# agnusmaximus/DistributedMNIST

Measured on AMD Instinct MI355X. Metric: images/sec (whole node), MNIST CNN sync-SGD, higher is better.
Workload: dtype bf16; 1 GPU; model=lenet, global_batch=1024, parallelism=dp1, mode=full_sync, mode_requested=full_sync, grad_dtype=fp32

## Files before the change

csrc/bindings.cpp:

```cpp

#include <torch/extension.h>
#include <ATen/hip/HIPContext.h>
#include <hip/hip_runtime.h>

#include "kernels.h"

namespace {

#define CHECK_BF16(t) TORCH_CHECK((t).scalar_type() == at::kBFloat16, #t " must be bf16")
#define CHECK_F32(t) TORCH_CHECK((t).scalar_type() == at::kFloat, #t " must be fp32")
#define CHECK_CONTIG(t) TORCH_CHECK((t).is_contiguous(), #t " must be contiguous")
#define CHECK_CUDA(t) TORCH_CHECK((t).is_cuda(), #t " must be on GPU")

const unsigned short* bf16_ptr(const torch::Tensor& t) {
  return reinterpret_cast<const unsigned short*>(t.data_ptr());
}
unsigned short* bf16_mut(torch::Tensor& t) {
  return reinterpret_cast<unsigned short*>(t.data_ptr());
}

hipStream_t cur_stream() {
  return at::hip::getCurrentHIPStream().stream();
}

int cdiv(int a, int b) { return (a + b - 1) / b; }

int pick_splitk(int mtiles, int ntiles, int ksteps) {
  int tiles = mtiles * ntiles;
  if (tiles >= 256 || ksteps <= 1) return 1;
  int want = std::min(ksteps, std::max(1, 512 / tiles));
  return want;
}

int dw_tr_level() {
  static int v = [] {
    const char* e = getenv("DMNIST_DW_TR");
    return e ? atoi(e) : 1;
  }();
  return v;
}
bool dw_tr_enabled() { return dw_tr_level() != 0; }

bool conv2_dw_slab_route(int H, int W, int Cin, int Cout) {
  return conv2_dw_slab_supported(H, W, Cin, Cout) && dw_tr_enabled() &&
         conv2_dw_slab_enabled() && !getenv("DMNIST_DW_SPREAD");
}

torch::Tensor linear_act_fwd_impl(torch::Tensor x, torch::Tensor w,
                                  torch::Tensor b, bool relu, double p_keep,
                                  int64_t seed, int64_t offset,
                                  const long* offset_dev,
                                  const c10::optional<torch::Tensor>& wT) {
  CHECK_CUDA(x); CHECK_BF16(x); CHECK_CONTIG(x);
  CHECK_BF16(w); CHECK_CONTIG(w);
  CHECK_F32(b); CHECK_CONTIG(b);
  int M = x.size(0), K = x.size(1), N = w.size(1);
  TORCH_CHECK(w.size(0) == K, "w/x shape mismatch");
  auto y = torch::empty({M, N}, x.options());
  GemmParams p{};
  p.A = bf16_ptr(x);
  p.bias = b.data_ptr<float>();
  p.C = y.data_ptr(); p.amax = nullptr;
  p.M = M; p.N = N; p.K = K;
  p.lda = K; p.ldc = N;
  p.splitk = 1;
  p.p_keep = (float)p_keep; p.seed = (uint64_t)seed; p.offset = (uint64_t)offset;
  p.offset_dev = offset_dev;
  bool drop = p_keep < 1.0;
  TORCH_CHECK(!drop || relu, "dropout path requires relu epilogue");
  int g128 = cdiv(M, 128) * cdiv(N, 128);
  bool big = g128 >= 512;
  if (const char* e = getenv("DMNIST_FC_TILE")) big = atoi(e) >= 128;
  auto s = cur_stream();
  bool bt = wT.has_value() && wT->defined();
  int tiles64 = cdiv(M, 64) * cdiv(N, 64);
  int ksteps = cdiv(K, 64);
  if (!big && tiles64 < 256 && ksteps >= 16 &&
      !getenv("DMNIST_FC_NOSPLIT")) {
    int sk = std::min(ksteps, std::max(2, 512 / tiles64));
    auto acc = torch::empty({(int64_t)sk, (int64_t)M, (int64_t)N},
                            x.options().dtype(at::kFloat));
    p.C = acc.data_ptr();
    p.splitk = sk;
    if (bt) {
      CHECK_BF16((*wT)); CHECK_CONTIG((*wT));
      TORCH_CHECK(wT->size(0) == N && wT->size(1) == K, "wT shape mismatch");
      p.B = bf16_ptr(*wT); p.ldb = K;
      gemm_fwd_slices_64_bt(p, s);
    } else {
      p.B = bf16_ptr(w); p.ldb = N;
      gemm_fwd_slices_64(p, s);
    }
    launch_fwd_epilogue(acc.data_ptr<float>(), b.data_ptr<float>(),
                        bf16_mut(y), M, N, sk, relu ? 1 : 0, (float)p_keep,
                        (uint64_t)seed, (uint64_t)offset, offset_dev, s);
    return y;
  }
  if (bt) {
    CHECK_BF16((*wT)); CHECK_CONTIG((*wT));
    TORCH_CHECK(wT->size(0) == N && wT->size(1) == K, "wT shape mismatch");
    p.B = bf16_ptr(*wT); p.ldb = K;
    if (drop) (big ? gemm_fwd_drop_128_bt : gemm_fwd_drop_64_bt)(p, s);
    else if (relu) (big ? gemm_fwd_relu_128_bt : gemm_fwd_relu_64_bt)(p, s);
    else (big ? gemm_fwd_bias_128_bt : gemm_fwd_bias_64_bt)(p, s);
  } else {
    p.B = bf16_ptr(w); p.ldb = N;
    if (drop) (big ? gemm_fwd_drop_128 : gemm_fwd_drop_64)(p, s);
    else if (relu) (big ? gemm_fwd_relu_128 : gemm_fwd_relu_64)(p, s);
    else (big ? gemm_fwd_bias_128 : gemm_fwd_bias_64)(p, s);
  }
  return y;
}

torch::Tensor linear_act_fwd(torch::Tensor x, torch::Tensor w, torch::Tensor b,
                             bool relu, double p_keep, int64_t seed,
                             int64_t offset,
                             c10::optional<torch::Tensor> wT) {
  return linear_act_fwd_impl(x, w, b, relu, p_keep, seed, offset, nullptr, wT);
// ... 24 lines not shown
  CHECK_F32(db); CHECK_CONTIG(db);
  torch::Tensor dyeff;
  bool mask = relu || p_keep < 1.0;
  if (mask) {
    dyeff = torch::empty_like(dy);
    launch_relu_drop_bwd(bf16_ptr(dy), bf16_ptr(y), bf16_mut(dyeff),
                         db.data_ptr<float>(), B, N,
                         (float)(1.0 / p_keep), 1, s);
  } else {
    dyeff = dy;
    launch_relu_drop_bwd(bf16_ptr(dy), bf16_ptr(y), bf16_mut(dyeff),
                         db.data_ptr<float>(), B, N, 1.0f, 0, s);
  }
  if (!dw.defined())
    dw = torch::zeros({K, N}, x.options().dtype(at::kFloat));
  CHECK_F32(dw); CHECK_CONTIG(dw);
  {
    GemmParams p{};
    p.A = bf16_ptr(x); p.B = bf16_ptr(dyeff);
    p.C = dw.data_ptr();
    p.M = K; p.N = N; p.K = B;
    p.lda = K;
    p.ldb = N; p.ldc = N;
    if (dw_tr_enabled() && K % 8 == 0 && N % 64 == 0) {
      int bn = (N % 128 == 0) ? 128 : 64;
      p.splitk = pick_splitk(cdiv(K, 128), cdiv(N, bn), cdiv(B, 32));
      (bn == 128 ? gemm_dw_tr_128 : gemm_dw_tr_64)(p, s);
    } else {
      bool big = cdiv(K, 128) * cdiv(N, 128) >= 128;
      int bm = big ? 128 : 64;
      p.splitk = pick_splitk(cdiv(K, bm), cdiv(N, bm), cdiv(B, 32));
      (big ? gemm_dw_128 : gemm_dw_64)(p, s);
    }
  }
  torch::Tensor dx;
  if (need_dx) {
    dx = torch::empty({B, K}, x.options());
    GemmParams p{};
    p.A = bf16_ptr(dyeff); p.B = bf16_ptr(w);
    p.C = dx.data_ptr();
    p.M = B; p.N = K; p.K = N;
    p.lda = N; p.ldb = N; p.ldc = K;
    p.splitk = 1;
    bool big = cdiv(B, 128) * cdiv(K, 128) >= 128;
    (big ? gemm_dx_128 : gemm_dx_64)(p, s);
  } else {
    dx = torch::empty({0}, x.options());
  }
  return {dx, dw, db};
}

std::vector<torch::Tensor> linear_act_bwd(torch::Tensor dy, torch::Tensor x,
                                          torch::Tensor w, torch::Tensor y,
                                          bool relu, double p_keep,
                                          bool need_dx) {
  return linear_act_bwd_impl(dy, x, w, y, relu, p_keep, need_dx,
// ... 156 lines not shown
                      double p_keep, torch::Tensor db_out) {
  CHECK_CUDA(dy); CHECK_BF16(dy); CHECK_CONTIG(dy);
  CHECK_F32(db_out); CHECK_CONTIG(db_out);
  int B = dy.size(0), N = dy.size(1);
  auto s = cur_stream();
  bool mask = relu || p_keep < 1.0;
  torch::Tensor dyeff = mask ? torch::empty_like(dy) : dy;
  launch_relu_drop_bwd(bf16_ptr(dy), mask ? bf16_ptr(y) : bf16_ptr(dy),
                       bf16_mut(dyeff), db_out.data_ptr<float>(), B, N,
                       (float)(1.0 / p_keep), mask ? 1 : 0, s);
  return dyeff;
}

void linear_dw_into(torch::Tensor x, torch::Tensor dyeff,
                    torch::Tensor dw_out) {
  CHECK_BF16(x); CHECK_CONTIG(x); CHECK_BF16(dyeff); CHECK_CONTIG(dyeff);
  CHECK_F32(dw_out);
  int B = x.size(0), K = x.size(1), N = dyeff.size(1);
  GemmParams p{};
  p.A = bf16_ptr(x); p.B = bf16_ptr(dyeff);
  p.C = dw_out.data_ptr();
  p.M = K; p.N = N; p.K = B;
  p.lda = K; p.ldb = N; p.ldc = N;
  if (dw_tr_enabled() && K % 8 == 0 && N % 64 == 0) {
    int bn = (N % 128 == 0) ? 128 : 64;
    p.splitk = pick_splitk(cdiv(K, 128), cdiv(N, bn), cdiv(B, 32));
    (bn == 128 ? gemm_dw_tr_128 : gemm_dw_tr_64)(p, cur_stream());
    return;
  }
  bool big = cdiv(K, 128) * cdiv(N, 128) >= 128;
  int bm = big ? 128 : 64;
  p.splitk = pick_splitk(cdiv(K, bm), cdiv(N, bm), cdiv(B, 32));
  (big ? gemm_dw_128 : gemm_dw_64)(p, cur_stream());
}

torch::Tensor linear_dx(torch::Tensor dyeff, torch::Tensor w) {
  CHECK_BF16(dyeff); CHECK_CONTIG(dyeff); CHECK_BF16(w); CHECK_CONTIG(w);
  int B = dyeff.size(0), N = dyeff.size(1), K = w.size(0);
  auto dx = torch::empty({B, K}, dyeff.options());
  GemmParams p{};
  p.A = bf16_ptr(dyeff); p.B = bf16_ptr(w);
  p.C = dx.data_ptr();
  p.M = B; p.N = K; p.K = N;
  p.lda = N; p.ldb = N; p.ldc = K;
  p.splitk = 1;
  bool big = cdiv(B, 128) * cdiv(K, 128) >= 128;
  (big ? gemm_dx_128 : gemm_dx_64)(p, cur_stream());
  return dx;
}

torch::Tensor linear_dx_unpool(torch::Tensor dyeff, torch::Tensor w,
                               torch::Tensor amax, torch::Tensor db_out,
                               int64_t Ho, int64_t Wo, int64_t C) {
  CHECK_BF16(dyeff); CHECK_CONTIG(dyeff); CHECK_BF16(w); CHECK_CONTIG(w);
  int B = dyeff.size(0), N = dyeff.size(1), K = w.size(0);
  TORCH_CHECK(K == Ho * Wo * C, "linear_dx_unpool: K != Ho*Wo*C");
  auto dact = torch::empty({B, 2 * (int)Ho, 2 * (int)Wo, (int)C},
                           dyeff.options());
  GemmParams p{};
  p.A = bf16_ptr(dyeff); p.B = bf16_ptr(w);
  p.C = dact.data_ptr();
  p.M = B; p.N = K; p.K = N;
  p.lda = N; p.ldb = N; p.ldc = K;
  p.splitk = 1;
  p.CHo = Ho; p.CWo = Wo; p.Cout = C;
  p.amax = amax.data_ptr<uint8_t>();
  p.db = db_out.defined() ? db_out.data_ptr<float>() : nullptr;
  bool big = cdiv(B, 128) * cdiv(K, 128) >= 512;
  (big ? gemm_dx_unpool_128 : gemm_dx_unpool_64)(p, cur_stream());
  return dact;
}

torch::Tensor linear_dx_mask(torch::Tensor dyeff, torch::Tensor w,
                             torch::Tensor actm, torch::Tensor db_out,
                             double p_keep) {
  CHECK_BF16(dyeff); CHECK_CONTIG(dyeff); CHECK_BF16(w); CHECK_CONTIG(w);
  CHECK_BF16(actm); CHECK_CONTIG(actm);
  int B = dyeff.size(0), N = dyeff.size(1), K = w.size(0);
  TORCH_CHECK(actm.size(0) == B && actm.size(1) == K, "actm shape mismatch");
  auto dx = torch::empty({B, K}, dyeff.options());
  GemmParams p{};
  p.A = bf16_ptr(dyeff); p.B = bf16_ptr(w);
  p.C = dx.data_ptr();
  p.M = B; p.N = K; p.K = N;
  p.lda = N; p.ldb = N; p.ldc = K;
  p.splitk = 1;
  p.p_keep = (float)(1.0 / p_keep);
  p.actm = bf16_ptr(actm);
  p.db = db_out.defined() ? db_out.data_ptr<float>() : nullptr;
  bool big = cdiv(B, 128) * cdiv(K, 128) >= 128;
  (big ? gemm_dx_mask_128 : gemm_dx_mask_64)(p, cur_stream());
// ... 389 lines not shown
}

PYBIND11_MODULE(TORCH_EXTENSION_NAME, m) {
  m.def("linear_act_fwd", &linear_act_fwd, "fused linear+bias+relu+dropout",
        py::arg("x"), py::arg("w"), py::arg("b"), py::arg("relu"),
        py::arg("p_keep"), py::arg("seed"), py::arg("offset"),
        py::arg("wT") = c10::nullopt);
  m.def("transpose_bf16", &transpose_bf16, "bf16 2-D transpose (wT refresh)");
  m.def("transpose_bf16_batch_adv", &transpose_bf16_batch_adv,
        "batched transposes + fused device step/LR advance (graph tail)");
  m.def("transpose_bf16_batch", &transpose_bf16_batch,
        "up to 4 transposes in one launch");
  m.def("mask_db", &mask_db, "relu/dropout grad mask + bias-grad column sums");
  m.def("linear_dw_into", &linear_dw_into, "dW = x^T dyeff into bucket view");
  m.def("linear_dx", &linear_dx, "dx = dyeff @ W^T");
  m.def("linear_dx_mask", &linear_dx_mask,
        "dx GEMM with fused relu/dropout mask + bias-grad column sums",
        py::arg("dyeff"), py::arg("w"), py::arg("actm"), py::arg("db_out"),
        py::arg("p_keep"));
  m.def("linear_dx_unpool", &linear_dx_unpool,
        "dx GEMM fused with maxpool2x2 backward scatter + conv db",
        py::arg("dyeff"), py::arg("w"), py::arg("amax"),
        py::arg("db_out"), py::arg("Ho"), py::arg("Wo"), py::arg("C"));
  m.def("pool_scatter", &pool_scatter, "maxpool bwd scatter + conv db");
  m.def("conv_dw_into", &conv_dw_into, "conv dW into bucket view");
  m.def("conv1_dw_pooled", &conv1_dw_pooled,
        "conv1 dW+db from the pooled gradient (pool bwd fused, no dact1)",
        py::arg("x"), py::arg("dyp"), py::arg("am"),
        py::arg("dw_out"), py::arg("db_out"));
  m.def("conv1_dw_group", [](int64_t NB) {
          return (int64_t)conv1_mfma_dw_group((int)NB);
        }, "images per block the MFMA conv1 dW launcher picks for batch NB");
  m.def("conv2_dw_group", [](int64_t NB) {
          return (int64_t)conv2_dw_group((int)NB);
        }, "images per block the slab conv2 dW launcher picks for batch NB");
  m.def("conv_dx", &conv_dx, "conv dX");
  m.def("linear_act_bwd", &linear_act_bwd, "linear backward (dx, dw, db)");
  m.def("linear_act_bwd_into", &linear_act_bwd_into,
        "linear backward accumulating dw/db into bucket views");
  m.def("conv_pool_fwd", &conv_pool_fwd, "fused conv5x5+bias+relu+maxpool",
        py::arg("x"), py::arg("w"), py::arg("b"), py::arg("wT") = c10::nullopt);
  m.def("conv_pool_bwd", &conv_pool_bwd, "conv+pool backward (dx, dw, db)");
  m.def("conv_pool_bwd_into", &conv_pool_bwd_into,
        "conv backward accumulating dw/db into bucket views");
  m.def("softmax_xent_fwd", &softmax_xent_fwd, "fused softmax-CE (+grad, +optional fc2 db, +optional acc-mean scale)",
        py::arg("logits"), py::arg("labels"),
// ... 51 lines not shown
```

csrc/dw_tr.hip:

```cpp

#include "common.h"
#include "kernels.h"

#define NT 256

__device__ __align__(16) unsigned short g_zero_page[8];

enum { AM_PLAIN = 0, AM_CONV5 = 1 };

template <int BN, int AMODE, int TBM = 128, int TBK = 64, int NBUF = 2>
__global__ __launch_bounds__(NT) void dw_tr_kernel(GemmParams p) {
  static_assert(TBK % 32 == 0, "TBK in 32-k MFMA halves");
  static_assert(NBUF == 2 || NBUF == 3, "2-buf overlap or 3-buf glds span");
  constexpr int WM = TBM / 2, WN = BN / 2;
  constexpr int MI = WM / 16, NI = WN / 16;
  constexpr int AQ = TBM * TBK / 2048;
  constexpr int BQ = BN * TBK / 2048;
  constexpr int ALPR = TBM / 8;
  constexpr int BLPR = BN / 8;
  __shared__ __align__(16) ushort_t Aimg[NBUF][TBK][TBM];
  __shared__ __align__(16) ushort_t Bimg[NBUF][TBK][BN];

  const int tid = threadIdx.x;
  const int lane = tid & 63;
  const int wave = tid >> 6;
  const int wr = wave >> 1, wc = wave & 1;

  int gx = (p.M + TBM - 1) / TBM;
  int gy = (p.N + BN - 1) / BN;
  int total = gx * gy * p.splitk;
  int flat = blockIdx.x;
  int q8 = total / 8, r8 = total % 8;
  int xcd = flat % 8, pos = flat / 8;
  int flat2 = (xcd < r8 ? xcd * (q8 + 1) : r8 * (q8 + 1) + (xcd - r8) * q8) + pos;
  const int m0 = (flat2 % gx) * TBM;
  int rest = flat2 / gx;
  const int n0 = (rest % gy) * BN;
  const int bz = rest / gy;

  int ksteps_total = (p.K + TBK - 1) / TBK;
  int steps_per = (ksteps_total + p.splitk - 1) / p.splitk;
  int kbeg = bz * steps_per * TBK;
  int kend = min(p.K, kbeg + steps_per * TBK);
  int nt = (kend - kbeg + TBK - 1) / TBK;
  if (nt < 0) nt = 0;

  f32x4 acc[MI][NI];
#pragma unroll
  for (int mi = 0; mi < MI; ++mi)
#pragma unroll
    for (int ni = 0; ni < NI; ++ni) acc[mi][ni] = f32x4{0.f, 0.f, 0.f, 0.f};

  int amc[AQ];
  bool am_ok[AQ];
  int akh[AQ], akw[AQ], aci[AQ];
#pragma unroll
  for (int q = 0; q < AQ; ++q) {
    int rt = (wave * AQ + q) * (512 / TBM) + lane / ALPR;
    int xs = (rt ^ (rt >> 4)) & (ALPR - 1);
    amc[q] = m0 + ((lane % ALPR) ^ xs) * 8;
    am_ok[q] = amc[q] < p.M;
    if (AMODE == AM_CONV5) {
      int khkw = amc[q] / p.Cin;
      aci[q] = amc[q] % p.Cin;
      akh[q] = khkw / 5 - 2;
      akw[q] = khkw % 5 - 2;
    } else {
      akh[q] = akw[q] = aci[q] = 0;
    }
  }
  int bnc[BQ];
  bool bn_ok[BQ];
#pragma unroll
  for (int q = 0; q < BQ; ++q) {
    int rt = (wave * BQ + q) * (512 / BN) + lane / BLPR;
    int xs = (rt ^ (rt >> 3)) & (BLPR - 1);
    bnc[q] = n0 + ((lane % BLPR) ^ xs) * 8;
    bn_ok[q] = bnc[q] < p.N;
  }

  int aw[AQ], ah[AQ], an[AQ];
  int dw64 = 0, dh64 = 0, dn64 = 0;
// ... 41 lines not shown
    for (int q = 0; q < BQ; ++q) {
      int gi = wave * BQ + q;
      int row0 = gi * (512 / BN);
      int k = kt + row0 + lane / BLPR;
      const ushort_t* src = (k < kend && bn_ok[q])
                                ? p.B + (size_t)k * p.ldb + bnc[q]
                                : g_zero_page;
      glds16(src, &Bimg[buf][row0][0]);
    }
  };

  const int slot_r = (lane & 15) >> 2;
  const int slot_c = (lane & 3) * 4;
  const int kgrp = (lane >> 4) * 8;

  const auto compute = [&](int buf) {
    unsigned abase = (unsigned)(uintptr_t)&Aimg[buf][0][0];
    unsigned bbase = (unsigned)(uintptr_t)&Bimg[buf][0][0];
#pragma unroll
    for (int kh2 = 0; kh2 < TBK / 32; ++kh2) {
      int krow = kh2 * 32 + kgrp + slot_r;
      short8 af[MI], bf[NI];
      const auto aswz = [&](int r, int cb) {
        int xs = (r ^ (r >> 4)) & (ALPR - 1);
        return abase + (unsigned)(r * (TBM * 2) + (((cb >> 4) ^ xs) << 4) +
                                  (cb & 15));
      };
      const auto bswz = [&](int r, int cb) {
        int xs = (r ^ (r >> 3)) & (BLPR - 1);
        return bbase + (unsigned)(r * (BN * 2) + (((cb >> 4) ^ xs) << 4) +
                                  (cb & 15));
      };
      uint2 ar[MI][2], br[NI][2];
#pragma unroll
      for (int mi = 0; mi < MI; ++mi) {
        int cb = (wr * WM + mi * 16 + slot_c) * 2;
        ar[mi][0] = tr16_issue(aswz(krow, cb));
        ar[mi][1] = tr16_issue(aswz(krow + 4, cb));
      }
#pragma unroll
      for (int ni = 0; ni < NI; ++ni) {
        int cb = (wc * WN + ni * 16 + slot_c) * 2;
        br[ni][0] = tr16_issue(bswz(krow, cb));
        br[ni][1] = tr16_issue(bswz(krow + 4, cb));
      }
#pragma unroll
      for (int mi = 0; mi < MI; ++mi) af[mi] = pack_wait(ar[mi][0], ar[mi][1]);
#pragma unroll
      for (int ni = 0; ni < NI; ++ni) bf[ni] = pack_wait(br[ni][0], br[ni][1]);
#pragma unroll
      for (int mi = 0; mi < MI; ++mi)
#pragma unroll
        for (int ni = 0; ni < NI; ++ni)
          acc[mi][ni] = __builtin_amdgcn_mfma_f32_16x16x32_bf16(
              af[mi], bf[ni], acc[mi][ni], 0, 0, 0);
    }
  };

  constexpr int INFLIGHT = AQ + BQ;
  if (NBUF == 3) {
    if (nt > 0) issue(0, kbeg);
    if (nt > 1) {
      issue(1 % NBUF, kbeg + TBK);
      asm volatile("s_waitcnt vmcnt(%0)" ::"i"(INFLIGHT) : "memory");
    } else {
      asm volatile("s_waitcnt vmcnt(0)" ::: "memory");
    }
    __builtin_amdgcn_s_barrier();
    for (int t = 0; t < nt; ++t) {
      if (t + 2 < nt) issue((t + 2) % NBUF, kbeg + (t + 2) * TBK);
      compute(t % NBUF);
      if (t + 2 < nt)
        asm volatile("s_waitcnt vmcnt(%0)" ::"i"(INFLIGHT) : "memory");
      else
        asm volatile("s_waitcnt vmcnt(0)" ::: "memory");
      __builtin_amdgcn_s_barrier();
    }
  } else {
    int cur = 0;
    if (nt > 0) issue(0, kbeg);
    asm volatile("s_waitcnt vmcnt(0)" ::: "memory");
    __syncthreads();
    for (int t = 0; t < nt; ++t) {
      if (t + 1 < nt) issue(cur ^ 1, kbeg + (t + 1) * TBK);
      compute(cur);
      __syncthreads();
      cur ^= 1;
    }
  }

  const int frow = (lane >> 4) * 4;
  const int fcol = lane & 15;
  float* outp = reinterpret_cast<float*>(p.C);
  if (p.offset) outp += (size_t)(bz & 15) * p.M * p.ldc;
#pragma unroll
  for (int mi = 0; mi < MI; ++mi) {
#pragma unroll
    for (int ni = 0; ni < NI; ++ni) {
      int gc = n0 + wc * WN + ni * 16 + fcol;
      if (gc >= p.N) continue;
#pragma unroll
      for (int r = 0; r < 4; ++r) {
        int gr = m0 + wr * WM + mi * 16 + frow + r;
        if (gr >= p.M) continue;
        atomicAdd(outp + (size_t)gr * p.ldc + gc, acc[mi][ni][r]);
      }
    }
  }
}

static inline int cdiv_h(int a, int b) { return (a + b - 1) / b; }

void conv_dw_tr(const GemmParams& p, hipStream_t s) {
  static int tbm = [] {
    const char* e = getenv("DMNIST_DW_TBM");
    return e ? atoi(e) : 128;
  }();
  static int tbk = [] {
    const char* e = getenv("DMNIST_DW_TBK");
    return e ? atoi(e) : 32;
  }();
  dim3 grid(cdiv_h(p.M, tbm >= 256 ? 256 : 128) * cdiv_h(p.N, 64) * p.splitk);
  if (tbm >= 256)
    hipLaunchKernelGGL((dw_tr_kernel<64, AM_CONV5, 256>), grid, dim3(NT), 0,
                       s, p);
  else if (tbk <= 32 && getenv("DMNIST_DW_SPAN"))
    hipLaunchKernelGGL((dw_tr_kernel<64, AM_CONV5, 128, 32, 3>), grid,
                       dim3(NT), 0, s, p);
  else if (tbk <= 32)
    hipLaunchKernelGGL((dw_tr_kernel<64, AM_CONV5, 128, 32>), grid, dim3(NT),
                       0, s, p);
  else
    hipLaunchKernelGGL((dw_tr_kernel<64, AM_CONV5, 128>), grid, dim3(NT), 0,
                       s, p);
}

void gemm_dw_tr_128(const GemmParams& p, hipStream_t s) {
  dim3 grid(cdiv_h(p.M, 128) * cdiv_h(p.N, 128) * p.splitk);
  hipLaunchKernelGGL((dw_tr_kernel<128, AM_PLAIN>), grid, dim3(NT), 0, s, p);
}

void gemm_dw_tr_64(const GemmParams& p, hipStream_t s) {
  dim3 grid(cdiv_h(p.M, 128) * cdiv_h(p.N, 64) * p.splitk);
  hipLaunchKernelGGL((dw_tr_kernel<64, AM_PLAIN>), grid, dim3(NT), 0, s, p);
}
```

csrc/gemm_tile.hip:

```cpp

#include "common.h"
#include "kernels.h"

enum AMode {
  A_N = 0,
  A_T = 1,
  A_CONV_FWD = 2,
  A_CONV1_FWD = 3,
  A_CONV_DX = 4,
  A_CONV_DW = 5,
};
enum BMode {
  B_KMAJ = 0,
  B_NMAJ = 1,
  B_CONV_DX_W = 2,
};
enum Epi { EPI_NONE = 0, EPI_BIAS = 1, EPI_BIAS_RELU = 2, EPI_BIAS_RELU_DROP = 3,
           EPI_POOL = 4, EPI_UNPOOL = 5, EPI_MASK_DB = 6 };
enum OutKind { OUT_BF16 = 0, OUT_F32_ATOMIC = 1, OUT_F32_SLICES = 2 };

#define NTHREADS 256
#define BK 64
#define LDK (BK + 8)

DEV short8 loadRow8(const ushort_t* p, int vcnt) {
  short8 v;
  if (vcnt >= 8 && ((uintptr_t)p & 15) == 0) {
    v = *reinterpret_cast<const short8*>(p);
  } else {
#pragma unroll
    for (int j = 0; j < 8; ++j) v[j] = (j < vcnt) ? (short)p[j] : (short)0;
  }
  return v;
}

DEV bool decode_pool_m(const GemmParams& p, int m, int& n, int& oy, int& ox) {
  int q = m >> 2, pos = m & 3;
  int wo = q % p.CWo;
  int t = q / p.CWo;
  int ho = t % p.CHo;
  n = t / p.CHo;
  oy = ho * 2 + (pos >> 1);
// ... 153 lines not shown
    if (BMODE == B_KMAJ) {
      int kk = c / (BN / 8);
      int j0 = (c % (BN / 8)) * 8;
#pragma unroll
      for (int e = 0; e < 8; ++e) Bs[j0 + e][kk] = regs[j][e];
    } else {
      int i = c / (BK / 8);
      int kc = (c % (BK / 8)) * 8;
      *reinterpret_cast<short8*>(&Bs[i][kc]) = regs[j];
    }
  }
}

template <int BM, int BN, int AMODE, int BMODE, int EPI, int OUT, int PIPE,
          int SWZ = 0>
__global__ __launch_bounds__(NTHREADS)
void gemm_tile_kernel(GemmParams p) {
  constexpr int WM = BM / 2, WN = BN / 2;
  constexpr int MI = WM / 16, NI = WN / 16;
  constexpr int CHA = (BM * BK / 8) / NTHREADS;
  constexpr int CHB = (BN * BK / 8) / NTHREADS;
  constexpr int DB = (PIPE == 1) ? 2 : 1;
  static_assert(CHA >= 1 && CHB >= 1, "tile too small for 256 threads");
  __shared__ __align__(16) ushort_t As[DB][BM][LDK];
  __shared__ __align__(16) ushort_t Bs[DB][BN][LDK];
  constexpr bool HAS_DB = (EPI == EPI_UNPOOL || EPI == EPI_MASK_DB);
  __shared__ float dbred[HAS_DB ? BN : 1];
  if (HAS_DB && threadIdx.x < BN) dbred[threadIdx.x] = 0.f;

  const int tid = threadIdx.x;
  const int lane = tid & 63;
  const int wave = tid >> 6;
  const int wr = wave >> 1, wc = wave & 1;
  int bx = blockIdx.x, by = blockIdx.y, bz = blockIdx.z;
  if (SWZ) {
    int gx = (p.M + BM - 1) / BM;
    int gy = (p.N + BN - 1) / BN;
    int total = gx * gy * p.splitk;
    int flat = blockIdx.x;
    int q = total / 8, r = total % 8;
    int xcd = flat % 8, pos = flat / 8;
    int flat2 = (xcd < r ? xcd * (q + 1) : r * (q + 1) + (xcd - r) * q) + pos;
    bx = flat2 % gx;
    int rest = flat2 / gx;
    by = rest % gy;
    bz = rest / gy;
  }
  const int m0 = bx * BM;
  const int n0 = by * BN;

  int ksteps_total = (p.K + BK - 1) / BK;
  int steps_per = (ksteps_total + p.splitk - 1) / p.splitk;
  int kbeg = bz * steps_per * BK;
// ... 95 lines not shown
        for (int ni = 0; ni < NI; ++ni)
          acc[mi][ni] = __builtin_amdgcn_mfma_f32_16x16x32_bf16(
              af[mi], bf[ni], acc[mi][ni], 0, 0, 0);
    }
    if (PIPE) {
      if (have_next) {
        writeA<BM, AMODE, CHA>(As[cur ^ 1], tid, ra);
        writeB<BN, BMODE, CHB>(Bs[cur ^ 1], tid, rb);
        __syncthreads();
        cur ^= 1;
      }
    } else {
      __syncthreads();
    }
  }

epilogue:
  const int frow = (lane >> 4) * 4;
  const int fcol = lane & 15;
  float dbloc[(EPI == EPI_UNPOOL || EPI == EPI_MASK_DB) ? NI : 1];
  if (EPI == EPI_UNPOOL || EPI == EPI_MASK_DB)
#pragma unroll
    for (int ni = 0; ni < NI; ++ni) dbloc[ni] = 0.f;
#pragma unroll
  for (int mi = 0; mi < MI; ++mi) {
#pragma unroll
    for (int ni = 0; ni < NI; ++ni) {
      int gc = n0 + wc * WN + ni * 16 + fcol;
      if (gc >= p.N) continue;
      if (EPI == EPI_UNPOOL) {
        int c = gc % p.Cout;
        int pix = gc / p.Cout;
        int wo = pix % p.CWo, ho = pix / p.CWo;
        ushort_t* dact = reinterpret_cast<ushort_t*>(p.C);
        const int H2 = p.CHo * 2, W2 = p.CWo * 2;
#pragma unroll
        for (int r = 0; r < 4; ++r) {
          int gr = m0 + wr * WM + mi * 16 + frow + r;
          if (gr >= p.M) continue;
          size_t qoff = (size_t)gr * p.N + gc;
          int pos = p.amax[qoff];
          float g = pos < 4 ? acc[mi][ni][r] : 0.f;
          dbloc[ni] += g;
          ushort_t gb = f2bf(g);
#pragma unroll
          for (int rr = 0; rr < 2; ++rr)
// ... 23 lines not shown
        if (p.amax)
          p.amax[(size_t)gq * p.ldc + gc] = (uint8_t)(best > 0.f ? barg : 7);
      } else {
#pragma unroll
        for (int r = 0; r < 4; ++r) {
          int gr = m0 + wr * WM + mi * 16 + frow + r;
          if (gr >= p.M) continue;
          float v = acc[mi][ni][r];
          if (EPI == EPI_MASK_DB) {
            float a = bf2f(p.actm[(size_t)gr * p.ldc + gc]);
            v = (a > 0.f) ? v * p.p_keep : 0.f;
            dbloc[ni] += v;
          }
          if (EPI != EPI_NONE && EPI != EPI_MASK_DB) v += bias_v;
          if (EPI == EPI_BIAS_RELU || EPI == EPI_BIAS_RELU_DROP)
            v = v > 0.f ? v : 0.f;
          if (EPI == EPI_BIAS_RELU_DROP) {
            uint64_t off = p.offset_dev ? (uint64_t)*p.offset_dev : p.offset;
            float u = philox_uniform(p.seed, off, (uint64_t)gr * p.N + gc);
            v = (u < p.p_keep) ? v / p.p_keep : 0.f;
          }
          if (OUT == OUT_BF16) {
            reinterpret_cast<ushort_t*>(p.C)[(size_t)gr * p.ldc + gc] = f2bf(v);
          } else if (OUT == OUT_F32_SLICES) {
            float* outp = reinterpret_cast<float*>(p.C) +
                          (size_t)bz * p.M * p.ldc;
            outp[(size_t)gr * p.ldc + gc] = v;
          } else {
            atomicAdd(reinterpret_cast<float*>(p.C) + (size_t)gr * p.ldc + gc, v);
          }
        }
      }
    }
  }
  if (EPI == EPI_UNPOOL || EPI == EPI_MASK_DB) {
#pragma unroll
    for (int ni = 0; ni < NI; ++ni) {
      int colb = wc * WN + ni * 16 + fcol;
      if (dbloc[ni] != 0.f) atomicAdd(&dbred[colb], dbloc[ni]);
    }
    __syncthreads();
    if (p.db && (int)threadIdx.x < BN) {
      int gc = n0 + (int)threadIdx.x;
      float v = dbred[threadIdx.x];
      int idx = (EPI == EPI_UNPOOL) ? gc % p.Cout : gc;
      if (gc < p.N && v != 0.f) atomicAdd(&p.db[idx], v);
    }
  }
}

#include <hip/hip_runtime_api.h>

static inline int cdiv_host(int a, int b) { return (a + b - 1) / b; }

// ... 13 lines not shown

GEMM_ENTRY(gemm_fwd_bias_128, 128, 128, A_N, B_KMAJ, EPI_BIAS, OUT_BF16, 1)
GEMM_ENTRY(gemm_fwd_bias_64, 64, 64, A_N, B_KMAJ, EPI_BIAS, OUT_BF16, 1)
GEMM_ENTRY(gemm_fwd_relu_128, 128, 128, A_N, B_KMAJ, EPI_BIAS_RELU, OUT_BF16, 1)
GEMM_ENTRY(gemm_fwd_relu_64, 64, 64, A_N, B_KMAJ, EPI_BIAS_RELU, OUT_BF16, 1)
GEMM_ENTRY(gemm_fwd_drop_128, 128, 128, A_N, B_KMAJ, EPI_BIAS_RELU_DROP, OUT_BF16, 1)
GEMM_ENTRY(gemm_fwd_drop_64, 64, 64, A_N, B_KMAJ, EPI_BIAS_RELU_DROP, OUT_BF16, 1)
GEMM_ENTRY(gemm_dx_128, 128, 128, A_N, B_NMAJ, EPI_NONE, OUT_BF16, 1)
GEMM_ENTRY(gemm_dx_64, 64, 64, A_N, B_NMAJ, EPI_NONE, OUT_BF16, 1)
GEMM_ENTRY(gemm_dx_unpool_128, 128, 128, A_N, B_NMAJ, EPI_UNPOOL, OUT_BF16, 1)
GEMM_ENTRY(gemm_dx_unpool_64, 64, 64, A_N, B_NMAJ, EPI_UNPOOL, OUT_BF16, 1)
GEMM_ENTRY(gemm_dx_mask_128, 128, 128, A_N, B_NMAJ, EPI_MASK_DB, OUT_BF16, 1)
GEMM_ENTRY(gemm_dx_mask_64, 64, 64, A_N, B_NMAJ, EPI_MASK_DB, OUT_BF16, 1)
GEMM_ENTRY_SWZ(gemm_dw_128, 128, 128, A_T, B_KMAJ, EPI_NONE, OUT_F32_ATOMIC, 2)
GEMM_ENTRY_SWZ(gemm_dw_64, 64, 64, A_T, B_KMAJ, EPI_NONE, OUT_F32_ATOMIC, 2)
GEMM_ENTRY(gemm_fwd_bias_128_bt, 128, 128, A_N, B_NMAJ, EPI_BIAS, OUT_BF16, 1)
GEMM_ENTRY(gemm_fwd_bias_64_bt, 64, 64, A_N, B_NMAJ, EPI_BIAS, OUT_BF16, 1)
GEMM_ENTRY(gemm_fwd_relu_128_bt, 128, 128, A_N, B_NMAJ, EPI_BIAS_RELU, OUT_BF16, 1)
GEMM_ENTRY(gemm_fwd_relu_64_bt, 64, 64, A_N, B_NMAJ, EPI_BIAS_RELU, OUT_BF16, 1)
GEMM_ENTRY(gemm_fwd_drop_128_bt, 128, 128, A_N, B_NMAJ, EPI_BIAS_RELU_DROP, OUT_BF16, 1)
GEMM_ENTRY(gemm_fwd_drop_64_bt, 64, 64, A_N, B_NMAJ, EPI_BIAS_RELU_DROP, OUT_BF16, 1)
GEMM_ENTRY(gemm_fwd_slices_64, 64, 64, A_N, B_KMAJ, EPI_NONE, OUT_F32_SLICES, 1)
GEMM_ENTRY(gemm_fwd_slices_64_bt, 64, 64, A_N, B_NMAJ, EPI_NONE, OUT_F32_SLICES, 1)
GEMM_ENTRY(conv_fwd_pool, 128, 64, A_CONV_FWD, B_KMAJ, EPI_POOL, OUT_BF16, 0)
GEMM_ENTRY(conv_fwd_pool_bt, 128, 64, A_CONV_FWD, B_NMAJ, EPI_POOL, OUT_BF16, 0)
GEMM_ENTRY(conv1_fwd_pool, 128, 64, A_CONV1_FWD, B_KMAJ, EPI_POOL, OUT_BF16, 0)
GEMM_ENTRY(conv_dx_gemm, 128, 32, A_CONV_DX, B_CONV_DX_W, EPI_NONE, OUT_BF16, 0)
GEMM_ENTRY_SWZ(conv_dw_gemm, 128, 64, A_CONV_DW, B_KMAJ, EPI_NONE, OUT_F32_ATOMIC, 2)
GEMM_ENTRY_SWZ(conv1_dw_gemm, 32, 32, A_CONV_DW, B_KMAJ, EPI_NONE, OUT_F32_ATOMIC, 2)
```

csrc/kernels.h:

```cpp
#pragma once
#include <hip/hip_runtime.h>
#include <stdint.h>

struct GemmParams {
  const unsigned short* A;
  const unsigned short* B;
  const float* bias;
  void* C;
  uint8_t* amax;
  int M, N, K;
  int lda, ldb, ldc;
  int splitk;
  int CB, CH, CW, CHo, CWo, Cin, Cout;
  float p_keep;
  uint64_t seed, offset;
  const long* offset_dev;
  float* db;
  const unsigned short* actm;
};

void gemm_fwd_bias_128(const GemmParams&, hipStream_t);
void gemm_fwd_bias_64(const GemmParams&, hipStream_t);
void gemm_fwd_relu_128(const GemmParams&, hipStream_t);
void gemm_fwd_relu_64(const GemmParams&, hipStream_t);
void gemm_fwd_drop_128(const GemmParams&, hipStream_t);
void gemm_fwd_drop_64(const GemmParams&, hipStream_t);
void gemm_dx_128(const GemmParams&, hipStream_t);
void gemm_dx_64(const GemmParams&, hipStream_t);
void gemm_dx_unpool_128(const GemmParams&, hipStream_t);
void gemm_dx_unpool_64(const GemmParams&, hipStream_t);
void gemm_dx_mask_128(const GemmParams&, hipStream_t);
void gemm_dx_mask_64(const GemmParams&, hipStream_t);
void gemm_dw_128(const GemmParams&, hipStream_t);
void gemm_dw_64(const GemmParams&, hipStream_t);
void conv_fwd_pool(const GemmParams&, hipStream_t);
void conv1_fwd_pool(const GemmParams&, hipStream_t);
void conv_dx_gemm(const GemmParams&, hipStream_t);
void conv_dw_gemm(const GemmParams&, hipStream_t);
void conv_dw_tr(const GemmParams&, hipStream_t);
void gemm_dw_tr_128(const GemmParams&, hipStream_t);
void gemm_dw_tr_64(const GemmParams&, hipStream_t);

void launch_relu_drop_bwd(const unsigned short* dy, const unsigned short* y,
                          unsigned short* dyeff, float* db, int B, int N,
                          float inv_keep, int apply_mask, hipStream_t);
void launch_pool_bwd_scatter(const unsigned short* dy, const unsigned short* y,
                             const uint8_t* amax, unsigned short* dact,
                             float* db, int Mpool, int C, int H, int W, int Wo,
                             hipStream_t);
#define SOFTMAX_MAX_BLOCKS 4096
void launch_softmax_xent(const unsigned short* logits, const long* labels,
                         unsigned short* dlogits, float* out, int B, int C,
                         float* db, float inv_n, float* part,
                         unsigned* ticket, hipStream_t);
void launch_sgd_step(float* master, float* grad, unsigned short* shadow,
                     int has_shadow, long n, float lr_scale, float dc_keep,
                     uint64_t seed, uint64_t offset, float* momentum, float mu,
                     hipStream_t);
void launch_sgd_step_dev(float* master, float* grad,
                         unsigned short* shadow, int has_shadow, long n,
                         const float* lr_scale_dev, float dc_keep,
                         uint64_t seed, const long* offset_dev,
                         float* momentum, float mu, int zero_grad,
                         hipStream_t);
// ... 66 lines not shown
bool conv1_slab_supported(int H, int W, int Cin, int Cout);
void launch_conv1_dw_slab(const unsigned short* x, const unsigned short* dact,
                          float* dw, int NB, int H, int W, int Cout,
                          hipStream_t);
void launch_conv1_dw_direct(const unsigned short* x,
                            const unsigned short* dact, float* dw, int NB,
                            int H, int W, int Cout, hipStream_t s);
bool conv1_mfma_supported(int H, int W, int Cin, int Cout);
bool conv1_mfma_enabled();
int conv1_mfma_dw_group(int NB);
void launch_conv1_mfma_fwd(const unsigned short* x, const unsigned short* w,
                           const float* bias, unsigned short* y,
                           uint8_t* amax, int NB, hipStream_t);
void launch_conv1_mfma_dw(const unsigned short* x, const unsigned short* dyp,
                          const uint8_t* am, float* dw, float* db, int NB,
                          hipStream_t);
bool conv2_dw_slab_supported(int H, int W, int Cin, int Cout);
bool conv2_dw_slab_enabled();
int conv2_dw_group(int NB);
void launch_conv2_dw_slab(const unsigned short* x, const unsigned short* dact,
                          float* dw, int NB, hipStream_t);
void gemm_fwd_slices_64(const GemmParams&, hipStream_t);
void gemm_fwd_slices_64_bt(const GemmParams&, hipStream_t);
void launch_fwd_epilogue(const float* acc, const float* bias,
                         unsigned short* y, int M, int N, int slices,
                         int relu, float p_keep, uint64_t seed,
                         uint64_t offset, const long* offset_dev,
                         hipStream_t);
```

Measured before the change: 3.635 million images/sec.

## Retune fc dW tiling, add split-K fixup and line-based unpool scatter

Adds a dW planner that picks 64-row tiles and a smaller split-K for the fc weight-gradient GEMM, along with a single-writer MFMA-swapped variant that does vectorised read-modify-write instead of atomics. The unpool dx epilogue now stages gradients in LDS and writes full 16-byte lines into the upsampled activation gradient rather than scattering element by element. An opt-in split-K forward path uses per-tile tickets so the last block reduces the slices and applies the epilogue, removing a separate kernel. The changes add complexity and carry risks from swizzle changes and the ticket workspace handling.

Measured after the change: 3.812 million images/sec, median of 6. 4.9% higher.

```diff
diff --git a/csrc/bindings.cpp b/csrc/bindings.cpp
--- a/csrc/bindings.cpp
+++ b/csrc/bindings.cpp
@@ -30,6 +30,12 @@
   if (tiles >= 256 || ksteps <= 1) return 1;
   int want = std::min(ksteps, std::max(1, 512 / tiles));
   return want;
+}
+
+int clamp_splitk(int want, int ksteps) {
+  int s = std::max(1, std::min(want, ksteps));
+  int per = cdiv(ksteps, s);
+  return cdiv(ksteps, per);
 }
 
 int dw_tr_level() {
@@ -44,6 +50,44 @@
 bool conv2_dw_slab_route(int H, int W, int Cin, int Cout) {
   return conv2_dw_slab_supported(H, W, Cin, Cout) && dw_tr_enabled() &&
          conv2_dw_slab_enabled() && !getenv("DMNIST_DW_SPREAD");
+}
+
+struct DwPlan { int tr, tbm, bn, splitk; };
+DwPlan linear_dw_plan(int K, int N, int B) {
+  const int ksteps = cdiv(B, 64);
+  if (!(dw_tr_enabled() && K % 8 == 0 && N % 64 == 0)) {
+    int bm = cdiv(K, 128) * cdiv(N, 128) >= 128 ? 128 : 64;
+    int want = pick_splitk(cdiv(K, bm), cdiv(N, bm), cdiv(B, 32));
+    return {0, bm, bm, clamp_splitk(want, ksteps)};
+  }
+  int bn = (N % 128 == 0) ? 128 : 64;
+  DwPlan old{1, 128, bn,
+             clamp_splitk(pick_splitk(cdiv(K, 128), cdiv(N, bn), cdiv(B, 32)),
+                          ksteps)};
+  if (const char* e = getenv("DMNIST_DW_PLAN")) {
+    int tbm = 0, fbn = 0, sk = 0;
+    if (sscanf(e, "%d,%d,%d", &tbm, &fbn, &sk) == 3 &&
+        (tbm == 64 || tbm == 128) && (fbn == 64 || fbn == 128) &&
+        N % fbn == 0)
+      return {1, tbm, fbn, clamp_splitk(sk, ksteps)};
+    return old;
+  }
+  if (cdiv(K, 64) * cdiv(N, 64) >= 256) {
+    if (B < 1536) return {1, 64, 64, 1};
+    if (B < 6144) return {1, 64, bn, clamp_splitk(2, ksteps)};
+  }
+  return old;
+}
+
+void launch_linear_dw(GemmParams& p, int K, int N, int B, hipStream_t s) {
+  DwPlan pl = linear_dw_plan(K, N, B);
+  p.splitk = pl.splitk;
+  if (pl.tr) {
+    bool sw = pl.splitk == 1 && ((uintptr_t)p.C & 15) == 0 && p.ldc % 4 == 0;
+    gemm_dw_tr(p, pl.tbm, pl.bn, sw, s);
+  } else {
+    (pl.tbm == 128 ? gemm_dw_128 : gemm_dw_64)(p, s);
+  }
 }
 
 torch::Tensor linear_act_fwd_impl(torch::Tensor x, torch::Tensor w,
@@ -82,18 +126,37 @@
                             x.options().dtype(at::kFloat));
     p.C = acc.data_ptr();
     p.splitk = sk;
+    const char* fe = getenv("DMNIST_FC_FIXUP");
+    bool fixup = fe && atoi(fe) != 0 && N % 8 == 0;
+    if (fixup) {
+      static std::vector<torch::Tensor>* ws = new std::vector<torch::Tensor>(64);
+      int dev = x.get_device();
+      TORCH_CHECK(dev >= 0 && dev < 64, "linear_act_fwd: bad device index");
+      if (!(*ws)[dev].defined()) {
+        hipStreamCaptureStatus cap = hipStreamCaptureStatusNone;
+        hipStreamIsCapturing(s, &cap);
+        TORCH_CHECK(cap == hipStreamCaptureStatusNone,
+                    "linear_act_fwd: first split-K call on a device allocates "
+                    "its ticket workspace and must run outside graph capture");
+        (*ws)[dev] = torch::zeros({256}, x.options().dtype(at::kInt));
+      }
+      p.tickets = reinterpret_cast<unsigned*>((*ws)[dev].data_ptr<int>());
+      p.Y = bf16_mut(y);
+      p.relu = relu ? 1 : 0;
+    }
     if (bt) {
       CHECK_BF16((*wT)); CHECK_CONTIG((*wT));
       TORCH_CHECK(wT->size(0) == N && wT->size(1) == K, "wT shape mismatch");
       p.B = bf16_ptr(*wT); p.ldb = K;
-      gemm_fwd_slices_64_bt(p, s);
+      (fixup ? gemm_fwd_slices_fix_64_bt : gemm_fwd_slices_64_bt)(p, s);
     } else {
       p.B = bf16_ptr(w); p.ldb = N;
-      gemm_fwd_slices_64(p, s);
+      (fixup ? gemm_fwd_slices_fix_64 : gemm_fwd_slices_64)(p, s);
     }
-    launch_fwd_epilogue(acc.data_ptr<float>(), b.data_ptr<float>(),
-                        bf16_mut(y), M, N, sk, relu ? 1 : 0, (float)p_keep,
-                        (uint64_t)seed, (uint64_t)offset, offset_dev, s);
+    if (!fixup)
+      launch_fwd_epilogue(acc.data_ptr<float>(), b.data_ptr<float>(),
+                          bf16_mut(y), M, N, sk, relu ? 1 : 0, (float)p_keep,
+                          (uint64_t)seed, (uint64_t)offset, offset_dev, s);
     return y;
   }
   if (bt) {
@@ -164,16 +227,7 @@
     p.M = K; p.N = N; p.K = B;
     p.lda = K;
     p.ldb = N; p.ldc = N;
-    if (dw_tr_enabled() && K % 8 == 0 && N % 64 == 0) {
-      int bn = (N % 128 == 0) ? 128 : 64;
-      p.splitk = pick_splitk(cdiv(K, 128), cdiv(N, bn), cdiv(B, 32));
-      (bn == 128 ? gemm_dw_tr_128 : gemm_dw_tr_64)(p, s);
-    } else {
-      bool big = cdiv(K, 128) * cdiv(N, 128) >= 128;
-      int bm = big ? 128 : 64;
-      p.splitk = pick_splitk(cdiv(K, bm), cdiv(N, bm), cdiv(B, 32));
-      (big ? gemm_dw_128 : gemm_dw_64)(p, s);
-    }
+    launch_linear_dw(p, K, N, B, s);
   }
   torch::Tensor dx;
   if (need_dx) {
@@ -376,16 +430,7 @@
   p.C = dw_out.data_ptr();
   p.M = K; p.N = N; p.K = B;
   p.lda = K; p.ldb = N; p.ldc = N;
-  if (dw_tr_enabled() && K % 8 == 0 && N % 64 == 0) {
-    int bn = (N % 128 == 0) ? 128 : 64;
-    p.splitk = pick_splitk(cdiv(K, 128), cdiv(N, bn), cdiv(B, 32));
-    (bn == 128 ? gemm_dw_tr_128 : gemm_dw_tr_64)(p, cur_stream());
-    return;
-  }
-  bool big = cdiv(K, 128) * cdiv(N, 128) >= 128;
-  int bm = big ? 128 : 64;
-  p.splitk = pick_splitk(cdiv(K, bm), cdiv(N, bm), cdiv(B, 32));
-  (big ? gemm_dw_128 : gemm_dw_64)(p, cur_stream());
+  launch_linear_dw(p, K, N, B, cur_stream());
 }
 
 torch::Tensor linear_dx(torch::Tensor dyeff, torch::Tensor w) {
@@ -420,7 +465,11 @@
   p.CHo = Ho; p.CWo = Wo; p.Cout = C;
   p.amax = amax.data_ptr<uint8_t>();
   p.db = db_out.defined() ? db_out.data_ptr<float>() : nullptr;
-  bool big = cdiv(B, 128) * cdiv(K, 128) >= 512;
+  const char* le = getenv("DMNIST_UNPOOL_LINES");
+  p.unpool_lines = !(le && atoi(le) == 0) && C % 64 == 0 &&
+                   ((uintptr_t)p.amax & 15) == 0 && ((uintptr_t)p.C & 15) == 0;
+  bool big = cdiv(B, 128) * cdiv(K, 128) >= (p.unpool_lines ? 400 : 512);
+  if (const char* e = getenv("DMNIST_UNPOOL_TILE")) big = atoi(e) >= 128;
   (big ? gemm_dx_unpool_128 : gemm_dx_unpool_64)(p, cur_stream());
   return dact;
 }
@@ -856,6 +905,10 @@
         "dx GEMM fused with maxpool2x2 backward scatter + conv db",
         py::arg("dyeff"), py::arg("w"), py::arg("amax"),
         py::arg("db_out"), py::arg("Ho"), py::arg("Wo"), py::arg("C"));
+  m.def("linear_dw_plan", [](int64_t K, int64_t N, int64_t B) {
+    DwPlan pl = linear_dw_plan((int)K, (int)N, (int)B);
+    return std::make_tuple(pl.tbm, pl.bn, pl.splitk);
+  }, "(tbm, bn, splitk) the fc dW launcher picks for x[B,K], dyeff[B,N]");
   m.def("pool_scatter", &pool_scatter, "maxpool bwd scatter + conv db");
   m.def("conv_dw_into", &conv_dw_into, "conv dW into bucket view");
   m.def("conv1_dw_pooled", &conv1_dw_pooled,
diff --git a/csrc/dw_tr.hip b/csrc/dw_tr.hip
--- a/csrc/dw_tr.hip
+++ b/csrc/dw_tr.hip
@@ -8,7 +8,8 @@
 
 enum { AM_PLAIN = 0, AM_CONV5 = 1 };
 
-template <int BN, int AMODE, int TBM = 128, int TBK = 64, int NBUF = 2>
+template <int BN, int AMODE, int TBM = 128, int TBK = 64, int NBUF = 2,
+          int SW = 0>
 __global__ __launch_bounds__(NT) void dw_tr_kernel(GemmParams p) {
   static_assert(TBK % 32 == 0, "TBK in 32-k MFMA halves");
   static_assert(NBUF == 2 || NBUF == 3, "2-buf overlap or 3-buf glds span");
@@ -51,13 +52,14 @@
 #pragma unroll
     for (int ni = 0; ni < NI; ++ni) acc[mi][ni] = f32x4{0.f, 0.f, 0.f, 0.f};
 
+  constexpr int ASH = (ALPR == 16) ? 4 : 3;
   int amc[AQ];
   bool am_ok[AQ];
   int akh[AQ], akw[AQ], aci[AQ];
 #pragma unroll
   for (int q = 0; q < AQ; ++q) {
     int rt = (wave * AQ + q) * (512 / TBM) + lane / ALPR;
-    int xs = (rt ^ (rt >> 4)) & (ALPR - 1);
+    int xs = (rt ^ (rt >> ASH)) & (ALPR - 1);
     amc[q] = m0 + ((lane % ALPR) ^ xs) * 8;
     am_ok[q] = amc[q] < p.M;
     if (AMODE == AM_CONV5) {
@@ -145,7 +147,7 @@
       int krow = kh2 * 32 + kgrp + slot_r;
       short8 af[MI], bf[NI];
       const auto aswz = [&](int r, int cb) {
-        int xs = (r ^ (r >> 4)) & (ALPR - 1);
+        int xs = (r ^ (r >> ASH)) & (ALPR - 1);
         return abase + (unsigned)(r * (TBM * 2) + (((cb >> 4) ^ xs) << 4) +
                                   (cb & 15));
       };
@@ -175,8 +177,10 @@
       for (int mi = 0; mi < MI; ++mi)
 #pragma unroll
         for (int ni = 0; ni < NI; ++ni)
-          acc[mi][ni] = __builtin_amdgcn_mfma_f32_16x16x32_bf16(
-              af[mi], bf[ni], acc[mi][ni], 0, 0, 0);
+          acc[mi][ni] = SW ? __builtin_amdgcn_mfma_f32_16x16x32_bf16(
+                                 bf[ni], af[mi], acc[mi][ni], 0, 0, 0)
+                           : __builtin_amdgcn_mfma_f32_16x16x32_bf16(
+                                 af[mi], bf[ni], acc[mi][ni], 0, 0, 0);
     }
   };
 
@@ -216,6 +220,21 @@
   const int fcol = lane & 15;
   float* outp = reinterpret_cast<float*>(p.C);
   if (p.offset) outp += (size_t)(bz & 15) * p.M * p.ldc;
+  if (SW) {
+#pragma unroll
+    for (int mi = 0; mi < MI; ++mi) {
+      int gr = m0 + wr * WM + mi * 16 + fcol;
+      if (gr >= p.M) continue;
+#pragma unroll
+      for (int ni = 0; ni < NI; ++ni) {
+        int gc = n0 + wc * WN + ni * 16 + frow;
+        if (gc >= p.N) continue;
+        f32x4* o = reinterpret_cast<f32x4*>(outp + (size_t)gr * p.ldc + gc);
+        *o = *o + acc[mi][ni];
+      }
+    }
+    return;
+  }
 #pragma unroll
   for (int mi = 0; mi < MI; ++mi) {
 #pragma unroll
@@ -258,12 +277,22 @@
                        s, p);
 }
 
-void gemm_dw_tr_128(const GemmParams& p, hipStream_t s) {
-  dim3 grid(cdiv_h(p.M, 128) * cdiv_h(p.N, 128) * p.splitk);
-  hipLaunchKernelGGL((dw_tr_kernel<128, AM_PLAIN>), grid, dim3(NT), 0, s, p);
-}
-
-void gemm_dw_tr_64(const GemmParams& p, hipStream_t s) {
-  dim3 grid(cdiv_h(p.M, 128) * cdiv_h(p.N, 64) * p.splitk);
-  hipLaunchKernelGGL((dw_tr_kernel<64, AM_PLAIN>), grid, dim3(NT), 0, s, p);
-}
+template <int BN, int TBM>
+static void dw_tr_plain(const GemmParams& p, bool sw, hipStream_t s) {
+  dim3 grid(cdiv_h(p.M, TBM) * cdiv_h(p.N, BN) * p.splitk);
+  if (sw)
+    hipLaunchKernelGGL((dw_tr_kernel<BN, AM_PLAIN, TBM, 64, 2, 1>), grid,
+                       dim3(NT), 0, s, p);
+  else
+    hipLaunchKernelGGL((dw_tr_kernel<BN, AM_PLAIN, TBM>), grid, dim3(NT), 0,
+                       s, p);
+}
+
+void gemm_dw_tr(const GemmParams& p, int tbm, int bn, bool single_writer,
+                hipStream_t s) {
+  bool sw = single_writer && p.splitk == 1;
+  if (tbm == 64)
+    (bn == 128 ? dw_tr_plain<128, 64> : dw_tr_plain<64, 64>)(p, sw, s);
+  else
+    (bn == 128 ? dw_tr_plain<128, 128> : dw_tr_plain<64, 128>)(p, sw, s);
+}
diff --git a/csrc/gemm_tile.hip b/csrc/gemm_tile.hip
--- a/csrc/gemm_tile.hip
+++ b/csrc/gemm_tile.hip
@@ -17,7 +17,8 @@
 };
 enum Epi { EPI_NONE = 0, EPI_BIAS = 1, EPI_BIAS_RELU = 2, EPI_BIAS_RELU_DROP = 3,
            EPI_POOL = 4, EPI_UNPOOL = 5, EPI_MASK_DB = 6 };
-enum OutKind { OUT_BF16 = 0, OUT_F32_ATOMIC = 1, OUT_F32_SLICES = 2 };
+enum OutKind { OUT_BF16 = 0, OUT_F32_ATOMIC = 1, OUT_F32_SLICES = 2,
+               OUT_F32_SLICES_FIX = 3 };
 
 #define NTHREADS 256
 #define BK 64
@@ -217,13 +218,34 @@
   constexpr int CHB = (BN * BK / 8) / NTHREADS;
   constexpr int DB = (PIPE == 1) ? 2 : 1;
   static_assert(CHA >= 1 && CHB >= 1, "tile too small for 256 threads");
-  __shared__ __align__(16) ushort_t As[DB][BM][LDK];
-  __shared__ __align__(16) ushort_t Bs[DB][BN][LDK];
+  constexpr int A_BYTES = DB * BM * LDK * 2, B_BYTES = DB * BN * LDK * 2;
+  __shared__ __align__(16) unsigned char smem[A_BYTES + B_BYTES];
+  ushort_t (*As)[BM][LDK] = reinterpret_cast<ushort_t (*)[BM][LDK]>(smem);
+  ushort_t (*Bs)[BN][LDK] =
+      reinterpret_cast<ushort_t (*)[BN][LDK]>(smem + A_BYTES);
   constexpr bool HAS_DB = (EPI == EPI_UNPOOL || EPI == EPI_MASK_DB);
   __shared__ float dbred[HAS_DB ? BN : 1];
   if (HAS_DB && threadIdx.x < BN) dbred[threadIdx.x] = 0.f;
 
   const int tid = threadIdx.x;
+  constexpr bool UNP = (EPI == EPI_UNPOOL) && (BN % 64 == 0) &&
+                       (BM * BN / 16) % NTHREADS == 0 && SWZ == 0;
+  constexpr int NAM = UNP ? (BM * BN / 16) / NTHREADS : 1;
+  const bool use_lines = UNP && p.unpool_lines;
+  uint4 amreg[NAM];
+  if (use_lines) {
+    const int am_m0 = blockIdx.x * BM, am_n0 = blockIdx.y * BN;
+#pragma unroll
+    for (int i = 0; i < NAM; ++i) {
+      int idx = tid + i * NTHREADS;
+      int gr = am_m0 + idx / (BN / 16);
+      int gc = am_n0 + (idx % (BN / 16)) * 16;
+      amreg[i] = uint4{0x07070707u, 0x07070707u, 0x07070707u, 0x07070707u};
+      if (gr < p.M && gc < p.N)
+        amreg[i] = *reinterpret_cast<const uint4*>(p.amax + (size_t)gr * p.N + gc);
+    }
+  }
+
   const int lane = tid & 63;
   const int wave = tid >> 6;
   const int wr = wave >> 1, wc = wave & 1;
@@ -365,6 +387,74 @@
   if (EPI == EPI_UNPOOL || EPI == EPI_MASK_DB)
 #pragma unroll
     for (int ni = 0; ni < NI; ++ni) dbloc[ni] = 0.f;
+  if constexpr (UNP) {
+    if (use_lines) {
+      constexpr int NJ = BN / 64;
+      constexpr int MPP = 2 / NJ;
+      constexpr int PR = MPP * 16;
+      constexpr int STG = 64 * 4 * 128;
+      static_assert(MI % MPP == 0, "passes cover whole mi groups");
+      static_assert(STG + BM * BN <= A_BYTES + B_BYTES, "staging fits LDS");
+      unsigned char* ams = smem + STG;
+      ushort_t* dact = reinterpret_cast<ushort_t*>(p.C);
+      const int H2 = p.CHo * 2, W2 = p.CWo * 2;
+      const int key = lane >> 4;
+      __syncthreads();
+#pragma unroll
+      for (int i = 0; i < NAM; ++i) {
+        int idx = tid + i * NTHREADS;
+        int row = idx / (BN / 16), ch = idx % (BN / 16);
+        *reinterpret_cast<uint4*>(ams + row * BN +
+                                  ((ch ^ ((row >> 2) & 3)) << 4)) = amreg[i];
+      }
+#pragma unroll
+      for (int pass = 0; pass < MI / MPP; ++pass) {
+        __syncthreads();
+#pragma unroll
+        for (int mm = 0; mm < MPP; ++mm) {
+          const int mi = pass * MPP + mm;
+#pragma unroll
+          for (int ni = 0; ni < NI; ++ni) {
+            const int colt = wc * WN + ni * 16 + fcol;
+            const int j = colt >> 6, c = colt & 63;
+#pragma unroll
+            for (int r = 0; r < 4; ++r) {
+              const int rowt = wr * WM + mi * 16 + frow + r;
+              const int lr = wr * PR + mm * 16 + frow + r;
+              int pos = ams[rowt * BN + (((colt >> 4) ^ key) << 4) + (colt & 15)];
+              float g = pos < 4 ? acc[mi][ni][r] : 0.f;
+              dbloc[ni] += g;
+              ushort_t gb = f2bf(g);
+              unsigned char* sp = smem + ((lr * NJ + j) * 4) * 128 +
+                                  (((c >> 3) ^ (key << 1)) << 4) + (c & 7) * 2;
+#pragma unroll
+              for (int q = 0; q < 4; ++q)
+                *reinterpret_cast<ushort_t*>(sp + q * 128) =
+                    (pos == q) ? gb : (ushort_t)0;
+            }
+          }
+        }
+        __syncthreads();
+#pragma unroll
+        for (int i = 0; i < 8; ++i) {
+          int idx = tid + i * NTHREADS;
+          int ch = idx & 7, line = idx >> 3;
+          int q = line & 3, slot = line >> 2;
+          int j = slot % NJ, lr = slot / NJ;
+          int gr = m0 + (lr / PR) * WM + pass * PR + lr % PR;
+          int gcol = n0 + j * 64;
+          if (gr >= p.M || gcol >= p.N) continue;
+          int c0 = gcol % p.Cout, pix = gcol / p.Cout;
+          int wo = pix % p.CWo, ho = pix / p.CWo;
+          size_t o = (((size_t)gr * H2 + ho * 2 + (q >> 1)) * W2 + wo * 2 +
+                      (q & 1)) * p.Cout + c0 + ch * 8;
+          *reinterpret_cast<uint4*>(dact + o) = *reinterpret_cast<const uint4*>(
+              smem + (slot * 4 + q) * 128 + ((ch ^ (((lr >> 2) & 3) << 1)) << 4));
+        }
+      }
+    }
+  }
+  if (!use_lines) {
 #pragma unroll
   for (int mi = 0; mi < MI; ++mi) {
 #pragma unroll
@@ -434,14 +524,92 @@
           }
           if (OUT == OUT_BF16) {
             reinterpret_cast<ushort_t*>(p.C)[(size_t)gr * p.ldc + gc] = f2bf(v);
-          } else if (OUT == OUT_F32_SLICES) {
+          } else if (OUT == OUT_F32_SLICES || OUT == OUT_F32_SLICES_FIX) {
             float* outp = reinterpret_cast<float*>(p.C) +
                           (size_t)bz * p.M * p.ldc;
-            outp[(size_t)gr * p.ldc + gc] = v;
+            if (OUT == OUT_F32_SLICES_FIX)
+              __hip_atomic_store(&outp[(size_t)gr * p.ldc + gc], v,
+                                 __ATOMIC_RELAXED, __HIP_MEMORY_SCOPE_AGENT);
+            else
+              outp[(size_t)gr * p.ldc + gc] = v;
           } else {
             atomicAdd(reinterpret_cast<float*>(p.C) + (size_t)gr * p.ldc + gc, v);
           }
         }
+      }
+    }
+  }
+  }
+  if constexpr (OUT == OUT_F32_SLICES_FIX) {
+    static_assert(BM == 64 && BN == 64, "fix-up thread map is 64 x 64");
+    {
+      __shared__ unsigned last_flag;
+      __syncthreads();
+      unsigned* tk = p.tickets + (size_t)by * gridDim.x + bx;
+      if (tid == 0) {
+        __builtin_amdgcn_fence(__ATOMIC_RELEASE, "agent");
+        last_flag = (atomicAdd(tk, 1u) == (unsigned)p.splitk - 1u) ? 1u : 0u;
+      }
+      __syncthreads();
+      if (last_flag) {
+        __builtin_amdgcn_fence(__ATOMIC_ACQUIRE, "agent");
+        const size_t plane = (size_t)p.M * p.ldc;
+        const float* acc0 = reinterpret_cast<const float*>(p.C);
+        const uint64_t off = p.offset_dev ? (uint64_t)*p.offset_dev : p.offset;
+        const int gr = m0 + (tid >> 2);
+        const int gcb = n0 + (tid & 3) * 16;
+        const bool ok[2] = {gr < p.M && gcb < p.N, gr < p.M && gcb + 8 < p.N};
+        float sum[2][8];
+#pragma unroll
+        for (int h = 0; h < 2; ++h)
+#pragma unroll
+          for (int e = 0; e < 8; ++e) sum[h][e] = 0.f;
+        for (int s0 = 0; s0 < p.splitk; s0 += 4) {
+          union { unsigned long long q; float f[2]; } t[4][2][4];
+#pragma unroll
+          for (int ds = 0; ds < 4; ++ds)
+#pragma unroll
+            for (int h = 0; h < 2; ++h)
+#pragma unroll
+              for (int e2 = 0; e2 < 4; ++e2) {
+                t[ds][h][e2].q = 0ull;
+                if (ok[h] && s0 + ds < p.splitk)
+                  t[ds][h][e2].q = __hip_atomic_load(
+                      reinterpret_cast<const unsigned long long*>(
+                          acc0 + (size_t)(s0 + ds) * plane +
+                          (size_t)gr * p.N + gcb + h * 8 + e2 * 2),
+                      __ATOMIC_RELAXED, __HIP_MEMORY_SCOPE_AGENT);
+              }
+#pragma unroll
+          for (int ds = 0; ds < 4; ++ds)
+            if (s0 + ds < p.splitk)
+#pragma unroll
+              for (int h = 0; h < 2; ++h)
+#pragma unroll
+                for (int e = 0; e < 8; ++e)
+                  sum[h][e] += t[ds][h][e >> 1].f[e & 1];
+        }
+#pragma unroll
+        for (int h = 0; h < 2; ++h) {
+          const int gc = gcb + h * 8;
+          if (!ok[h]) continue;
+          union { ushort_t u[8]; uint4 v; } o;
+#pragma unroll
+          for (int e = 0; e < 8; ++e) {
+            const size_t i = (size_t)gr * p.N + gc + e;
+            float v = sum[h][e];
+            v += p.bias[gc + e];
+            if (p.relu) v = v > 0.f ? v : 0.f;
+            if (p.p_keep < 1.0f) {
+              float u = philox_uniform(p.seed, off, (uint64_t)i);
+              v = (u < p.p_keep) ? v / p.p_keep : 0.f;
+            }
+            o.u[e] = f2bf(v);
+          }
+          *reinterpret_cast<uint4*>(p.Y + (size_t)gr * p.N + gc) = o.v;
+        }
+        if (tid == 0)
+          __hip_atomic_store(tk, 0u, __ATOMIC_RELAXED, __HIP_MEMORY_SCOPE_AGENT);
       }
     }
   }
@@ -501,6 +669,8 @@
 GEMM_ENTRY(gemm_fwd_drop_64_bt, 64, 64, A_N, B_NMAJ, EPI_BIAS_RELU_DROP, OUT_BF16, 1)
 GEMM_ENTRY(gemm_fwd_slices_64, 64, 64, A_N, B_KMAJ, EPI_NONE, OUT_F32_SLICES, 1)
 GEMM_ENTRY(gemm_fwd_slices_64_bt, 64, 64, A_N, B_NMAJ, EPI_NONE, OUT_F32_SLICES, 1)
+GEMM_ENTRY(gemm_fwd_slices_fix_64, 64, 64, A_N, B_KMAJ, EPI_NONE, OUT_F32_SLICES_FIX, 1)
+GEMM_ENTRY(gemm_fwd_slices_fix_64_bt, 64, 64, A_N, B_NMAJ, EPI_NONE, OUT_F32_SLICES_FIX, 1)
 GEMM_ENTRY(conv_fwd_pool, 128, 64, A_CONV_FWD, B_KMAJ, EPI_POOL, OUT_BF16, 0)
 GEMM_ENTRY(conv_fwd_pool_bt, 128, 64, A_CONV_FWD, B_NMAJ, EPI_POOL, OUT_BF16, 0)
 GEMM_ENTRY(conv1_fwd_pool, 128, 64, A_CONV1_FWD, B_KMAJ, EPI_POOL, OUT_BF16, 0)
diff --git a/csrc/kernels.h b/csrc/kernels.h
--- a/csrc/kernels.h
+++ b/csrc/kernels.h
@@ -17,6 +17,10 @@
   const long* offset_dev;
   float* db;
   const unsigned short* actm;
+  int unpool_lines;
+  unsigned* tickets;
+  unsigned short* Y;
+  int relu;
 };
 
 void gemm_fwd_bias_128(const GemmParams&, hipStream_t);
@@ -38,8 +42,8 @@
 void conv_dx_gemm(const GemmParams&, hipStream_t);
 void conv_dw_gemm(const GemmParams&, hipStream_t);
 void conv_dw_tr(const GemmParams&, hipStream_t);
-void gemm_dw_tr_128(const GemmParams&, hipStream_t);
-void gemm_dw_tr_64(const GemmParams&, hipStream_t);
+void gemm_dw_tr(const GemmParams&, int tbm, int bn, bool single_writer,
+                hipStream_t);
 
 void launch_relu_drop_bwd(const unsigned short* dy, const unsigned short* y,
                           unsigned short* dyeff, float* db, int B, int N,
@@ -152,6 +156,8 @@
                           float* dw, int NB, hipStream_t);
 void gemm_fwd_slices_64(const GemmParams&, hipStream_t);
 void gemm_fwd_slices_64_bt(const GemmParams&, hipStream_t);
+void gemm_fwd_slices_fix_64(const GemmParams&, hipStream_t);
+void gemm_fwd_slices_fix_64_bt(const GemmParams&, hipStream_t);
 void launch_fwd_epilogue(const float* acc, const float* bias,
                          unsigned short* y, int M, int N, int slices,
                          int relu, float p_keep, uint64_t seed,
```
